# WardellZc/DeepLearningRecommendationSystem

Measured on AMD Instinct MI355X. Metric: CTR samples/sec fwd+bwd at batch 65536, higher is better.
Workload: dtype f32; 1 GPU; neuralcf mf_dim=64 layers=[128,64,32,16,8] users=943 items=1682 batch=65536/gpu (BASELINE configs[1]); global_batch=65536, parallelism=single

## Files before the change

### deeplearningrecommendationsystem_amd/csrc/ncf_proj.hip

```cpp
#include "ctr_common.h"

#include <stdlib.h>

namespace {

constexpr int kThreads = 256;
constexpr int kWaves = kThreads / 64;
constexpr int kL = 3;
constexpr int kK[kL] = {64, 32, 16};
constexpr int kN[kL] = {32, 16, 8};
constexpr int kH = 64;
constexpr int kN0 = 64;
constexpr int kP = 64;
constexpr int kNL = 8;
constexpr int kHeadW = kP + kNL;

#include "mfma16_tower.inc"

#ifdef CTR_STAMPS
__device__ unsigned long long g_stamps[2][64];
#define STAMP(k, i) do { const int at_ = (i); if (blockIdx.x == 7 && threadIdx.x == 0 && at_ < 64) g_stamps[k][at_] = __builtin_readcyclecounter(); } while (0)
#else
#define STAMP(k, i) do {} while (0)
#endif

struct Ids {
  const int64_t* uidx; int64_t ustride;
  const int64_t* iidx; int64_t istride;
  int64_t nu, ni;
};

constexpr int kChunks = 64;
constexpr int kPlanHead = 4;
static_assert(kPlanHead + 2 * (kChunks + 2) + 1 <= 2 * CTR_NCF_PROJ_COUNT_STRIDE,
              "CTR_NCF_PROJ_COUNT_STRIDE: the plan of the smallest tables (two rows) does not fit");
struct Plan {
  unsigned int* ticket;
  int32_t* base; int32_t* totals; int32_t* offsets;
  int64_t rows;
  int shift, chunks;
};
Plan plan_of(int32_t* buf, int64_t rows, int64_t m) {
  int shift = 8;
  while (((int64_t)kChunks << shift) < m) ++shift;
  Plan p;
  p.ticket = reinterpret_cast<unsigned int*>(buf);
  p.base = buf + kPlanHead;
  p.totals = p.base + kChunks * rows;
  p.offsets = p.totals + rows;
  p.rows = rows;
  p.shift = shift;
  p.chunks = (int)((m + ((int64_t)1 << shift) - 1) >> shift);
  return p;
}

struct RankJob {
  Ids ids;
  Plan plan; int32_t* ranks;
  int64_t m;
  int first;
};
constexpr int kRankPer = 4;
__device__ __forceinline__ void rank_role(const RankJob& R) {
  extern __shared__ __attribute__((aligned(16))) int s_hist[];
  const int chunk = (int)blockIdx.x - R.first;
  const int rows = (int)R.plan.rows;
  for (int i = threadIdx.x; i < rows; i += kThreads) s_hist[i] = 0;
  __syncthreads();
  const int64_t lo = (int64_t)chunk << R.plan.shift;
  const int64_t hi = lo + ((int64_t)1 << R.plan.shift) < R.m ? lo + ((int64_t)1 << R.plan.shift) : R.m;
  for (int64_t s0 = lo + threadIdx.x; s0 < hi; s0 += kRankPer * kThreads) {
    int64_t u[kRankPer], i[kRankPer];
#pragma unroll
    for (int e = 0; e < kRankPer; ++e) {
      const int64_t s = s0 + e * kThreads < hi ? s0 + e * kThreads : hi - 1;
      u[e] = R.ids.uidx[s * R.ids.ustride];
      i[e] = R.ids.iidx[s * R.ids.istride];
    }
#pragma unroll
    for (int e = 0; e < kRankPer; ++e) {
      const int64_t s = s0 + e * kThreads;
      if (s < hi) {
        int ru = -1, ri = -1;
        if ((uint64_t)u[e] < (uint64_t)R.ids.nu) ru = atomicAdd(s_hist + u[e], 1);
        if ((uint64_t)i[e] < (uint64_t)R.ids.ni) ri = atomicAdd(s_hist + R.ids.nu + i[e], 1);
        *reinterpret_cast<int2*>(R.ranks + 2 * s) = make_int2(ru, ri);
      }
    }
  }
  __syncthreads();
  int32_t* out = R.plan.base + (int64_t)chunk * rows;
  for (int i = threadIdx.x; i < rows; i += kThreads) out[i] = s_hist[i];
}

struct PlanJob {
  Plan plan;
  int first;
};
__device__ __forceinline__ void plan_role(const PlanJob& J, int* lds) {
  __shared__ int s_scan[kWaves];
  __shared__ bool s_last;
  const Plan& P = J.plan;
  const int64_t rows = P.rows;
  const int lane = threadIdx.x & 63, wave = threadIdx.x >> 6;
  {
    const int64_t row = ((int64_t)blockIdx.x - J.first) * kThreads + threadIdx.x;
    const int64_t rr = row < rows ? row : rows - 1;
    int v[kChunks];
#pragma unroll
    for (int c = 0; c < kChunks; ++c) v[c] = P.base[(int64_t)(c < P.chunks ? c : P.chunks - 1) * rows + rr];
    int run = 0;
#pragma unroll
    for (int c = 0; c < kChunks; ++c)
      if (c < P.chunks && row < rows) {
        P.base[(int64_t)c * rows + row] = run;
        run += v[c];
      }
    if (row < rows) __hip_atomic_store(P.totals + row, run, __ATOMIC_RELAXED, __HIP_MEMORY_SCOPE_AGENT);
  }
  __syncthreads();
  if (threadIdx.x == 0) {
    const unsigned int drawn = __hip_atomic_fetch_add(P.ticket, 1u, __ATOMIC_ACQ_REL, __HIP_MEMORY_SCOPE_AGENT);
    s_last = drawn == gridDim.x - (unsigned int)J.first - 1u;
  }
  __syncthreads();
  if (!s_last) return;
  constexpr int kCnt = 12;
  for (int64_t base = 0; base < rows; base += kCnt * kThreads) {
    int v[kCnt];
#pragma unroll
    for (int e = 0; e < kCnt; ++e) {
      const int64_t i = base + e * kThreads + threadIdx.x;
      v[e] = __hip_atomic_load(P.totals + (i < rows ? i : rows - 1), __ATOMIC_RELAXED, __HIP_MEMORY_SCOPE_AGENT);
    }
#pragma unroll
    for (int e = 0; e < kCnt; ++e) {
      const int64_t i = base + e * kThreads + threadIdx.x;
      if (i < rows) lds[i] = v[e];
    }
  }
  __syncthreads();
  const int per = (int)((rows + kThreads - 1) / kThreads);
  const int64_t i0 = (int64_t)threadIdx.x * per;
  int sum = 0;
  for (int e = 0; e < per; ++e)
    if (i0 + e < rows) sum += lds[i0 + e];
  int inc = sum;
#pragma unroll
  for (int d = 1; d < 64; d <<= 1) {
    const int v = __shfl_up(inc, d, 64);
    if (lane >= d) inc += v;
  }
  if (lane == 63) s_scan[wave] = inc;
  __syncthreads();
  int before = 0;
  for (int w = 0; w < wave; ++w) before += s_scan[w];
  int run = before + inc - sum;
  for (int e = 0; e < per; ++e)
    if (i0 + e < rows) {
      const int c = lds[i0 + e];
      lds[i0 + e] = run;
      run += c;
    }
  if (threadIdx.x == kThreads - 1) lds[rows] = before + inc;
  __syncthreads();
  for (int64_t i = threadIdx.x; i <= rows; i += kThreads) P.offsets[i] = lds[i];
  if (threadIdx.x == 0) __hip_atomic_store(P.ticket, 0u, __ATOMIC_RELAXED, __HIP_MEMORY_SCOPE_AGENT);
}

struct Prep {
  const float* mlp_u; const float* mlp_i;
  const float* w0; int64_t ldw0; const float* b0;
  float* ptab;
  int64_t nu, ni;
  const float* fold_u; const float* fold_w; int64_t fold_ldw; const float* fold_b; const float* fold_b2;
  float* wfold;
  RankJob rank;
};

__global__ void __launch_bounds__(kThreads)
ncfp_prep_kernel(const Prep A) {
  if ((int)blockIdx.x >= A.rank.first) {
    rank_role(A.rank);
    return;
  }
  const int lane = threadIdx.x & 63, q = lane >> 4, n = lane & 15;
  const int64_t wave = ((int64_t)blockIdx.x * kThreads + threadIdx.x) >> 6;
  const int64_t ublocks = (A.nu + 15) / 16, iblocks = (A.ni + 15) / 16;
  if ((int)blockIdx.x == A.rank.first - 1) {
    __shared__ float s_f[kThreads];
    const int t = threadIdx.x;
    const float* u = A.fold_u + kP;
    if (t < kP) A.wfold[t] = A.fold_u[t];
    {
      const int c = t & 7, i = t >> 3;
      s_f[t] = fmaf(A.fold_w[(int64_t)i * A.fold_ldw + c], u[i], A.fold_w[(int64_t)(i + 32) * A.fold_ldw + c] * u[i + 32]);
    }
    __syncthreads();
    if (t < kNL) {
      float acc = 0.0f;
      for (int i = 0; i < 32; ++i) acc += s_f[8 * i + t];
      A.wfold[kP + t] = acc;
    }
    __syncthreads();
    if (t < 64) s_f[t] = A.fold_b ? A.fold_b[t] * u[t] : 0.0f;
    __syncthreads();
    if (t == 0) {
      float acc = A.fold_b2 ? A.fold_b2[0] : 0.0f;
      for (int i = 0; i < 64; ++i) acc += s_f[i];
      A.wfold[kHeadW] = acc;
    }
  }
  if (wave >= ublocks + iblocks) return;
  const bool user = wave < ublocks;
  const int64_t row = (user ? wave : wave - ublocks) * 16 + n, rows = user ? A.nu : A.ni;
  const float* tab = user ? A.mlp_u : A.mlp_i;
  const int coff = user ? 0 : kH;
  const bool live = row < rows;
  f32x4 x[4], acc[4];
#pragma unroll
  for (int j = 0; j < 4; ++j) x[j] = ldg4(tab + (live ? row : 0) * kH + 16 * j + 4 * q);
#pragma unroll
  for (int b = 0; b < 4; ++b) {
    if (!user && A.b0) acc[b] = ldg4(A.b0 + 16 * b + 4 * q);
    else acc[b] = f32x4{0.f, 0.f, 0.f, 0.f};
  }
#pragma unroll
  for (int j = 0; j < 4; ++j) {
    f32x4 w[4];
#pragma unroll
    for (int b = 0; b < 4; ++b) w[b] = ldg4(A.w0 + (int64_t)(16 * b + n) * A.ldw0 + coff + 16 * j + 4 * q);
#pragma unroll
    for (int c = 0; c < 4; ++c)
#pragma unroll
      for (int b = 0; b < 4; ++b) acc[b] = __builtin_amdgcn_mfma_f32_16x16x4f32(w[b][c], x[j][c], acc[b], 0, 0, 0);
  }
  if (live) {
    float* dst = A.ptab + ((user ? 0 : A.nu) + row) * kN0 + 4 * q;
#pragma unroll
    for (int b = 0; b < 4; ++b) stg4(dst + 16 * b, acc[b]);
  }
}

struct Fwd {
  Ids ids;
  const float* ptab;
  const float* gmf_u; const float* gmf_i;
  const float* wfold;
  float* out; int64_t ldout; int act;
  int32_t* err_flag;
  PlanJob plan;
};

constexpr int kFwdStage = 4 * 16 * 64;
constexpr int kFwdStores = 5;

__global__ void __launch_bounds__(kThreads) __attribute__((amdgpu_waves_per_eu(2, 2)))
ncfp_fwd_kernel(const Tower T, int64_t m, const Fwd F) {
  extern __shared__ __attribute__((aligned(16))) float lds[];
  if ((int)blockIdx.x >= F.plan.first) {
    plan_role(F.plan, reinterpret_cast<int*>(lds));
    return;
  }
  float* s_w = lds;
  float* s_b = s_w + kWFloats;
  float* s_hw = s_b + kBFloats;
  const int lane = threadIdx.x & 63, q = lane >> 4, n = lane & 15;
  const int wave = __builtin_amdgcn_readfirstlane(threadIdx.x >> 6);
  float* stage = s_hw + 80 + wave * kFwdStage;
  const uint32_t stage_addr = ctr_lds_addr(stage);
  const int64_t groups = (m + 15) / 16;
  const int64_t wave0 = ((int64_t)blockIdx.x * kThreads + threadIdx.x) >> 6, nwaves = ((int64_t)F.plan.first * kThreads) >> 6;
  const uint32_t nu = (uint32_t)F.ids.nu, ni = (uint32_t)F.ids.ni;
  const float* tabs[4] = {F.ptab, F.ptab + F.ids.nu * kN0, F.gmf_u, F.gmf_i};
  int64_t idu = 0, idi = 0;
  auto issue_ids = [&](int64_t g) {
    int64_t row = g * 16 + n;
    row = row < m ? row : m - 1;
    idu = F.ids.uidx[row * F.ids.ustride];
    idi = F.ids.iidx[row * F.ids.istride];
  };
  auto issue_rows = [&](int64_t g) {
    const bool live = g * 16 + n < m;
    const bool ubad = (uint64_t)idu >= nu, ibad = (uint64_t)idi >= ni;
    const uint32_t u = ubad ? 0u : (uint32_t)idu, i = ibad ? 0u : (uint32_t)idi;
    if (live && (ubad || ibad) && F.err_flag) *F.err_flag = 1;
#pragma unroll
    for (int k = 0; k < 4; ++k) {
      const int r = 4 * k + q;
      const int src = (lane & 48) | r;
      const uint32_t ur = (uint32_t)__shfl((int)u, src, 64), ir = (uint32_t)__shfl((int)i, src, 64);
      const uint32_t col = 4u * (uint32_t)(n ^ r);
#pragma unroll
      for (int t = 0; t < 4; ++t) {
        const float* g_ = tabs[t] + ((t & 1) ? ir : ur) * 64u + col;
        ctr_dma16(g_, stage_addr + (uint32_t)((t * 16 + 4 * k) * 256));
      }
    }
  };
  auto staged = [&](int t, int j) {
    return *reinterpret_cast<const f32x4*>(stage + (t * 16 + n) * 64 + 4 * ((4 * j + q) ^ n));
  };
  int stamp = 0;
  (void)stamp;
  STAMP(0, stamp++);
  issue_ids(wave0);
  {
    f32x4 wv[kFStagePer];
    int wdst[kFStagePer];
    float bv;
    stage_forward_load(T, wv, wdst, bv);
    float hw = 0.0f;
    if (threadIdx.x <= kHeadW) hw = F.wfold[threadIdx.x];
    issue_rows(wave0);
    issue_ids(wave0 + nwaves);
    stage_forward_store(s_w, s_b, wv, wdst, bv);
    if (threadIdx.x <= kHeadW) s_hw[threadIdx.x] = hw;
  }
  __syncthreads();
  STAMP(0, stamp++);
  const float hc = s_hw[kHeadW];
  if (wave0 >= groups) return;
  asm volatile("s_waitcnt vmcnt(0)" ::: "memory");
  asm volatile("" : "+v"(idu), "+v"(idi));
  for (int64_t g = wave0; g < groups; g += nwaves) {
    const int64_t row = g * 16 + n;
    const int64_t srow = row < m ? row : m;
    f32x4 a0[4], xe[4];
#pragma unroll
    for (int j = 0; j < 4; ++j) {
      const f32x4 z = staged(0, j) + staged(1, j);
#pragma unroll
      for (int r = 0; r < 4; ++r) a0[j][r] = fmaxf(z[r], 0.0f);
    }
#pragma unroll
    for (int i = 0; i < 4; ++i)
      xe[i] = *reinterpret_cast<const f32x4*>(stage + (2 * 16 + n) * 64 + 4 * ((4 * q + i) ^ n)) *
              *reinterpret_cast<const f32x4*>(stage + (3 * 16 + n) * 64 + 4 * ((4 * q + i) ^ n));
    asm volatile("s_waitcnt lgkmcnt(0)" ::: "memory");
    STAMP(0, stamp++);
    issue_rows(g + nwaves);
    issue_ids(g + 2 * nwaves);
    STAMP(0, stamp++);
    f32x4 y1[2], y2[1], y3[1];
    layer_fwd<0, 4>(s_w, s_b, lane, q, a0, y1);
    layer_fwd<1, 2>(s_w, s_b, lane, q, y1, y2);
    layer_fwd<2, 1>(s_w, s_b, lane, q, y2, y3);
    STAMP(0, stamp++);
#pragma unroll
    for (int b = 0; b < 2; ++b) stg4(T.y[0] + srow * T.ldy[0] + 16 * b + 4 * q, y1[b]);
    stg4(T.y[1] + srow * T.ldy[1] + 4 * q, y2[0]);
    stg4(T.y[2] + (q < 2 ? srow : m) * T.ldy[2] + 4 * (q & 1), y3[0]);
    float dot = 0.0f;
#pragma unroll
    for (int i = 0; i < 4; ++i) {
      const f32x4 wv = *reinterpret_cast<const f32x4*>(s_hw + 16 * q + 4 * i);
      dot = fmaf(xe[i][0], wv[0], dot); dot = fmaf(xe[i][1], wv[1], dot);
      dot = fmaf(xe[i][2], wv[2], dot); dot = fmaf(xe[i][3], wv[3], dot);
    }
    {
      const f32x4 wv = *reinterpret_cast<const f32x4*>(s_hw + kP + 4 * (q & 1));
      float d2 = y3[0][0] * wv[0];
      d2 = fmaf(y3[0][1], wv[1], d2); d2 = fmaf(y3[0][2], wv[2], d2); d2 = fmaf(y3[0][3], wv[3], d2);
      dot += q < 2 ? d2 : 0.0f;
    }
    dot += __shfl_xor(dot, 16, 64);
    dot += __shfl_xor(dot, 32, 64);
    F.out[srow * F.ldout] = ctr_act(dot + hc, F.act);
    STAMP(0, stamp++);
    asm volatile("s_waitcnt vmcnt(%0)" ::"n"(kFwdStores) : "memory");
    asm volatile("" : "+v"(idu), "+v"(idi));
  }
}

constexpr int slab_w(int l) {
  int o = 0;
  for (int i = 0; i < l; ++i) o += kN[i] * kK[i] + kN[i];
  return o;
}
constexpr int kSlabHead = slab_w(kL);
constexpr int kVecs = 8 + 2 + 1;
constexpr int kSmall = 32 + 16 + 8 + 8 + 1;
constexpr int kCopy = kVecs * 256 + 68;
constexpr int kSlab = kCopy;
constexpr int kStripP = 3 * kTile;
constexpr int kSgPU = 0, kSgPI = 1024, kSgY1 = 2048, kSgY2 = 2560, kSgY3 = 2816, kBwdStage = 3072;
constexpr int kBwdLdsMax = 150 * 1024 / 4;
constexpr int64_t bwd_lds_floats(int64_t rows) {
  const int64_t main_f = kWFloats + kWaves * (kStripP + kBwdStage) + (rows + 1 + 3) / 4 * 4, copy_f = (int64_t)kWaves * kCopy;
  return main_f > copy_f ? main_f : copy_f;
}
static_assert(bwd_lds_floats(CTR_NCF_PROJ_MAX_ROWS) <= kBwdLdsMax, "CTR_NCF_PROJ_MAX_ROWS: the backward's offsets do not fit in LDS");
constexpr int kBwdDma = 12;
constexpr int kBwdStores = 6;

struct Bwd {
  Ids ids;
  const float* ptab;
  const float* wfold;
  const float* prob; int64_t ldp;
  const float* gprob; int64_t ldgp;
  int act;
  const int32_t* base;
  const int32_t* offsets;
  int shift;
  const int32_t* ranks;
  float* gz;
  float* aux;
  float* slabs;
  float* zero_a; int64_t zero_a_floats;
  float* zero_b; int64_t zero_b_floats;
};

__device__ __forceinline__ int sw1(int r) { return (r >> 1) & 7; }
__device__ __forceinline__ int sw2(int r) { return (r >> 2) & 3; }
__device__ __forceinline__ int sw3(int r) { return (r >> 3) & 1; }

__global__ void __launch_bounds__(kThreads)
ncfp_bwd_kernel(const Tower T, int64_t m, const Bwd B) {
  extern __shared__ __attribute__((aligned(16))) float lds[];
  __shared__ __attribute__((aligned(16))) float s_hw[kHeadW + 4];
  float* s_wt = lds;
  const int lane = threadIdx.x & 63, q = lane >> 4, lo = lane & 15;
  const int wave = __builtin_amdgcn_readfirstlane(threadIdx.x >> 6);
  float* tA = lds + kWFloats + wave * kStripP;
  float* tB = tA + 2 * kTile;
  float* stage = lds + kWFloats + kWaves * kStripP + wave * kBwdStage;
  const uint32_t stage_addr = ctr_lds_addr(stage);
  const int64_t nrows = B.ids.nu + B.ids.ni;
  int* s_off = reinterpret_cast<int*>(lds + kWFloats + kWaves * (kStripP + kBwdStage));
  const int64_t groups = (m + 15) / 16;
  const int64_t wave0 = ((int64_t)blockIdx.x * kThreads + threadIdx.x) >> 6, nwaves = ((int64_t)gridDim.x * kThreads) >> 6;
  const f32x4 zero4 = {0.f, 0.f, 0.f, 0.f};
  const float* pu = B.ptab;
  const float* pi = B.ptab + B.ids.nu * kN0;
  const uint32_t nu = (uint32_t)B.ids.nu, ni = (uint32_t)B.ids.ni;
  int stamp = 0;
  (void)stamp;
  STAMP(1, stamp++);

  {
    const int64_t t0 = ((int64_t)blockIdx.x * kThreads + threadIdx.x) * 4, step = (int64_t)gridDim.x * kThreads * 4;
    for (int64_t i = t0; i < B.zero_a_floats; i += step) stg4(B.zero_a + i, zero4);
    if (B.zero_b)
      for (int64_t i = t0; i < B.zero_b_floats; i += step) stg4(B.zero_b + i, zero4);
  }
  int64_t idu = 0, idi = 0;
  auto issue_ids = [&](int64_t g) {
    int64_t row = g * 16 + lo;
    row = row < m ? row : m - 1;
    idu = B.ids.uidx[row * B.ids.ustride];
    idi = B.ids.iidx[row * B.ids.istride];
  };
  struct Scal {
    float gp, pb;
    int ru, ri;
    int bu, bi;
    uint32_t u, i;
    bool ubad, ibad;
  };
  auto issue_rows = [&](int64_t g, Scal& r) {
    int64_t rc = g * 16 + lo;
    rc = rc < m ? rc : m - 1;
    r.ubad = (uint64_t)idu >= nu;
    r.ibad = (uint64_t)idi >= ni;
    r.u = r.ubad ? 0u : (uint32_t)idu;
    r.i = r.ibad ? 0u : (uint32_t)idi;
#pragma unroll
    for (int k = 0; k < 4; ++k) {
      const int row = 4 * k + q;
      const int src = (lane & 48) | row;
      const uint32_t ur = (uint32_t)__shfl((int)r.u, src, 64), ir = (uint32_t)__shfl((int)r.i, src, 64);
      const uint32_t col = 4u * (uint32_t)(lo ^ row);
      ctr_dma16(pu + ur * 64u + col, stage_addr + (uint32_t)((kSgPU + 4 * k * 64) * 4));
      ctr_dma16(pi + ir * 64u + col, stage_addr + (uint32_t)((kSgPI + 4 * k * 64) * 4));
    }
    {
      const int64_t g16 = g * 16;
#pragma unroll
      for (int k = 0; k < 2; ++k) {
        const int row = 8 * k + (lane >> 3);
        int64_t gr = g16 + row;
        gr = gr < m ? gr : m - 1;
        ctr_dma16(T.y[0] + gr * T.ldy[0] + 4 * ((lane & 7) ^ sw1(row)), stage_addr + (uint32_t)((kSgY1 + 8 * k * 32) * 4));
      }
      {
        const int row = lane >> 2;
        int64_t gr = g16 + row;
        gr = gr < m ? gr : m - 1;
        ctr_dma16(T.y[1] + gr * T.ldy[1] + 4 * ((lane & 3) ^ sw2(row)), stage_addr + (uint32_t)(kSgY2 * 4));
      }
      {
        const int row = (lane >> 1) & 15;
        int64_t gr = g16 + row;
        gr = gr < m ? gr : m - 1;
        ctr_dma16(T.y[2] + gr * T.ldy[2] + 4 * ((lane & 1) ^ sw3(row)), stage_addr + (uint32_t)(kSgY3 * 4));
      }
    }
    r.gp = B.gprob[rc * B.ldgp];
    r.pb = B.prob[rc * B.ldp];
    r.ru = B.ranks[2 * rc];
    r.ri = B.ranks[2 * rc + 1];
    const int32_t* bc = B.base + (rc >> B.shift) * nrows;
    r.bu = bc[r.u];
    r.bi = bc[nu + r.i];
  };
  Scal sc;
  f32x4 dw0[2][4], dw1[2], dw2;
  f32x4 sb0[2], sb1, sb2, hy = zero4;
  float hc = 0.0f;
#pragma unroll
  for (int b = 0; b < 2; ++b) {
    sb0[b] = zero4;
    dw1[b] = zero4;
#pragma unroll
    for (int j = 0; j < 4; ++j) dw0[b][j] = zero4;
  }
  sb1 = sb2 = dw2 = zero4;
  issue_ids(wave0);
  {
    f32x4 wv[kStagePer];
    int wdst[kStagePer];
    stage_transposed_load(T, wv, wdst);
    const float hw = threadIdx.x <= kHeadW ? B.wfold[threadIdx.x] : 0.0f;
    constexpr int kCnt = 12;
    for (int64_t base = 0; base <= nrows; base += kCnt * kThreads) {
      int v[kCnt];
#pragma unroll
      for (int e = 0; e < kCnt; ++e) {
        const int64_t i = base + e * kThreads + threadIdx.x;
        v[e] = B.offsets[i <= nrows ? i : nrows];
      }
#pragma unroll
      for (int e = 0; e < kCnt; ++e) {
        const int64_t i = base + e * kThreads + threadIdx.x;
        if (i <= nrows) s_off[i] = v[e];
      }
    }
    issue_rows(wave0, sc);
// ... 193 lines not shown
    for (int u = 0; u < 7; ++u) tail[u] = src[(int64_t)(p + 8 * u < A.parts ? p + 8 * u : A.parts - 1) * kSlab];
#pragma unroll
    for (int u = 0; u < 7; ++u) acc[0] += (p + 8 * u < A.parts ? 1.0f : 0.0f) * tail[u];
  }
  float t = ((acc[0] + acc[1]) + (acc[2] + acc[3])) + ((acc[4] + acc[5]) + (acc[6] + acc[7]));
  t += __shfl_xor(t, 32, 64);
  if ((threadIdx.x & 63) < 32) s_part[wave][o] = t;
  __syncthreads();
  if (threadIdx.x < 32 && e < kSlabHead) {
    const float total = (s_part[0][o] + s_part[1][o]) + (s_part[2][o] + s_part[3][o]);
    int l = 0, r = e;
#pragma unroll
    for (int i = 0; i < kL; ++i)
      if (e >= slab_w(i)) { l = i; r = e - slab_w(i); }
    const int wn = l == 0 ? kN[0] * kK[0] : l == 1 ? kN[1] * kK[1] : kN[2] * kK[2];
    float* dst = r < wn ? A.gw[l] + r : A.gb[l] + (r - wn);
    dst[0] += total;
  }
}

__device__ __forceinline__ void head_fold_role(const Seg& A) {
  __shared__ float s_p[28][12];
  __shared__ float s_g[12];
  const int col = threadIdx.x % 9, pl = threadIdx.x / 9;
  float acc = 0.0f;
  if (pl < 28) {
    const float* src = A.slabs + kVecs * 256 + 56 + col;
    float v[10];
#pragma unroll
    for (int u = 0; u < 10; ++u) v[u] = 0.0f;
    for (int p0 = pl; p0 < A.parts; p0 += 28 * 10) {
      float x[10];
#pragma unroll
      for (int u = 0; u < 10; ++u) x[u] = src[(int64_t)(p0 + 28 * u < A.parts ? p0 + 28 * u : A.parts - 1) * kSlab];
#pragma unroll
      for (int u = 0; u < 10; ++u) v[u] += (p0 + 28 * u < A.parts ? 1.0f : 0.0f) * x[u];
    }
#pragma unroll
    for (int u = 0; u < 10; ++u) acc += v[u];
    s_p[pl][col] = acc;
  }
  __syncthreads();
  if (threadIdx.x < 9) {
    float t = 0.0f;
    for (int i = 0; i < 28; ++i) t += s_p[i][threadIdx.x];
    s_g[threadIdx.x] = t;
  }
  __syncthreads();
  const float* u = A.fold_u + kP;
  const float gc = s_g[kNL];
  for (int t = threadIdx.x; t < 64 * kNL; t += kThreads) {
    const int i = t / kNL, q = t % kNL;
    if (A.g_w) A.g_w[(int64_t)i * A.ld_g_w + q] += u[i] * s_g[q];
  }
  if (threadIdx.x < 64) {
    const int i = threadIdx.x;
    if (A.g_u) {
      float sacc = A.fold_b ? A.fold_b[i] * gc : 0.0f;
#pragma unroll
      for (int q = 0; q < kNL; ++q) sacc = fmaf(A.fold_w[(int64_t)i * A.fold_ldw + q], s_g[q], sacc);
      A.g_u[kP + i] += sacc;
    }
    if (A.g_b) A.g_b[i] += u[i] * gc;
  }
  if (threadIdx.x == 64 && A.g_b2) A.g_b2[0] += gc;
}

constexpr int kSegSlots = 16;
constexpr int kSegGroups = kThreads / 16;
constexpr int kSegWgSlots = kSegGroups * kSegSlots;
constexpr int kSegOpenL = 1, kSegOpenR = 2;

__global__ void __launch_bounds__(kThreads, 3)
ncfp_segsum_kernel(const Seg A) {
  if ((int)blockIdx.x >= A.seg_blocks) {
    if ((int)blockIdx.x < A.seg_blocks + A.red_blocks) slab_reduce_role(A, (int)blockIdx.x - A.seg_blocks);
    else head_fold_role(A);
    return;
  }
  __shared__ __attribute__((aligned(16))) float s_run[2 * kSegGroups][128];
  __shared__ int s_meta[2 * kSegGroups];
  const int lane = threadIdx.x & 63, lo = lane & 15, grp = threadIdx.x >> 4;
  const int64_t s0 = ((int64_t)blockIdx.x * kSegGroups + grp) * kSegSlots, sme = s0 + lo;
  const int64_t spare = 2 * A.m;
  const int64_t total = A.offsets[A.nu + A.ni];
  const f32x4 rec = ldg4(A.aux + (sme < spare ? sme : spare) * 4);
  const int64_t sb = s0 > 0 ? s0 - 1 : 0, sa = s0 + kSegSlots;
  const int row_before = __float_as_int(A.aux[(sb < spare ? sb : spare) * 4 + 2]);
  const int row_after = __float_as_int(A.aux[(sa < spare ? sa : spare) * 4 + 2]);
  const bool used = sme < total;
  const float gzv = used ? rec[0] : 0.0f;
  const int v = used && (uint32_t)__float_as_int(rec[2]) < (uint32_t)(A.nu + A.ni) ? __float_as_int(rec[2]) : -1;
  const bool urow = v < A.nu;
  const uint32_t pid = used ? min((uint32_t)__float_as_int(rec[1]), (uint32_t)((urow ? A.ni : A.nu) - 1)) : 0u;
  const int pk = (int)(2u * pid + (urow ? 1u : 0u));
  const uint32_t b = used ? min((uint32_t)__float_as_int(rec[3]), (uint32_t)A.m) : (uint32_t)A.m;
  const int v_before = (s0 > 0 && s0 - 1 < total) ? row_before : -1;
  const int v_after = sa < total ? row_after : -1;
  f32x4 g[kSegSlots], p[kSegSlots];
#pragma unroll
  for (int k = 0; k < kSegSlots; ++k) {
    const int src = (lane & 48) | k;
    const uint32_t bk = (uint32_t)__shfl((int)b, src, 64);
    const int pkk = __shfl(pk, src, 64);
    g[k] = ldg4(A.gz + (int64_t)bk * kN0 + 4 * lo);
    p[k] = ldg4(((pkk & 1) ? A.gmf_i : A.gmf_u) + (int64_t)(pkk >> 1) * kP + 4 * lo);
  }
  const f32x4 zero4 = {0.f, 0.f, 0.f, 0.f};
  f32x4 accs = zero4, acct = zero4;
  int cur = -1;
  bool inside = false;
  int meta0 = -1, meta1 = -1;
  auto store_run = [&](int r) {
    float* dst = A.st + (int64_t)r * 128;
    stg4(dst + 4 * lo, accs);
    stg4(dst + 64 + 4 * lo, acct);
  };
  auto park = [&](int e) {
    *reinterpret_cast<f32x4*>(&s_run[2 * grp + e][4 * lo]) = accs;
    *reinterpret_cast<f32x4*>(&s_run[2 * grp + e][64 + 4 * lo]) = acct;
  };
#pragma unroll
  for (int k = 0; k < kSegSlots; ++k) {
    const int src = (lane & 48) | k;
    const int vk = __shfl(v, src, 64);
    const float gk = __shfl(gzv, src, 64);
    if (vk != cur) {
      if (cur >= 0) {
        if (inside) store_run(cur);
        else {
          park(0);
          meta0 = (cur << 2) | kSegOpenL;
        }
      }
      inside = k > 0 || vk != v_before;
      cur = vk;
      accs = acct = zero4;
    }
    accs += g[k];
    acct += gk * p[k];
  }
  if (cur >= 0) {
    const bool open_r = cur == v_after;
    if (inside && !open_r) store_run(cur);
    else {
      park(1);
      meta1 = (cur << 2) | (inside ? 0 : kSegOpenL) | (open_r ? kSegOpenR : 0);
    }
  }
  if (lo == 0) {
    s_meta[2 * grp] = meta0;
    s_meta[2 * grp + 1] = meta1;
  }
  __syncthreads();
  if (threadIdx.x >= 128) return;
  const int c = threadIdx.x;
  float sum = 0.0f;
  int row = -1;
  bool shared = false;
  auto emit = [&](bool atomic) {
    float* dst = A.st + (int64_t)row * 128 + c;
    if (atomic) ctr_atomic_add_global(dst, sum);
    else dst[0] = sum;
    row = -1;
  };
  int meta[2 * kSegGroups];
  float val[2 * kSegGroups];
#pragma unroll
  for (int e = 0; e < 2 * kSegGroups; ++e) {
    meta[e] = s_meta[e];
    val[e] = s_run[e][c];
  }
  asm volatile("" ::: "memory");
#pragma unroll
  for (int e = 0; e < 2 * kSegGroups; ++e) {
    const int mt = __builtin_amdgcn_readfirstlane(meta[e]);
    const float x = val[e];
    if (mt >= 0) {
      const int r = mt >> 2;
      if (row >= 0 && r != row) emit(true);
      if (row < 0) {
        row = r;
        sum = 0.0f;
        shared = (mt & kSegOpenL) != 0;
      }
      sum += x;
      if (!(mt & kSegOpenR)) emit(shared);
    }
  }
  if (row >= 0) emit(true);
}

struct Fin {
  const float* st;
  const float* mlp_u; const float* mlp_i; const float* gmf_u; const float* gmf_i;
  const float* w0; int64_t ldw0;
  const float* wfold;
  int64_t nu, ni;
  float* g_mlp_u; float* g_mlp_i; float* g_gmf_u; float* g_gmf_i;
  float* g_w0; int64_t ldgw0; float* g_b0;
  float* g_head;
  int wgs;
};
constexpr int kFinParts = 4;

__global__ void __launch_bounds__(kThreads)
ncfp_finish_kernel(const Fin A) {
  __shared__ __attribute__((aligned(16))) float s_dw[2][8 * 256];
  __shared__ float s_sm[kWaves][2][64];
  const int lane = threadIdx.x & 63, q = lane >> 4, n = lane & 15, wave = threadIdx.x >> 6;
  const int part = (int)blockIdx.x / A.wgs, wg = (int)blockIdx.x - part * A.wgs, h = part & 1;
  const int64_t ublocks = (A.nu + 15) / 16, iblocks = (A.ni + 15) / 16;
  const int64_t uwgs = (ublocks + kWaves - 1) / kWaves;
  const bool user = wg < uwgs;
  const int64_t blk = (user ? (int64_t)wg : (int64_t)wg - uwgs) * kWaves + wave;
  const int64_t rows = user ? A.nu : A.ni, r0 = blk * 16;
  const bool any = blk < (user ? ublocks : iblocks);
  const float* st = A.st + (user ? 0 : A.nu) * 128;
  const float* tab = user ? A.mlp_u : A.mlp_i;
  const float* gmf = user ? A.gmf_u : A.gmf_i;
  float* gtab = user ? A.g_mlp_u : A.g_mlp_i;
  float* ggmf = user ? A.g_gmf_u : A.g_gmf_i;
  const int coff = user ? 0 : kH;
  const f32x4 zero4 = {0.f, 0.f, 0.f, 0.f};
  const int64_t row = r0 + n;
  const bool live = any && row < rows;
  const int64_t crow = live ? row : rows - 1;
  const float keep = live ? 1.0f : 0.0f;

  if (part >= 2) {
    if (!any || (!gtab && !ggmf)) return;
    f32x4 sd[4], td[2], og[2], ot[2], wf[2];
    const float* ogp = ggmf ? ggmf : gmf;
    const float* otp = gtab ? gtab : tab;
#pragma unroll
    for (int j = 0; j < 4; ++j) sd[j] = ldg4(st + crow * 128 + 16 * j + 4 * q);
#pragma unroll
    for (int e = 0; e < 2; ++e) {
      const int col = 16 * (2 * h + e) + 4 * q;
      td[e] = ldg4(st + crow * 128 + 64 + col);
      og[e] = ldg4(ogp + crow * kP + col);
      ot[e] = ldg4(otp + crow * kH + col);
      wf[e] = ldg4(A.wfold + col);
    }
    f32x4 wt[4][2];
#pragma unroll
    for (int c = 0; c < 4; ++c)
#pragma unroll
      for (int e = 0; e < 2; ++e)
#pragma unroll
        for (int j = 0; j < 4; ++j) wt[j][e][c] = A.w0[(int64_t)(16 * j + 4 * q + c) * A.ldw0 + coff + 16 * (2 * h + e) + n];
    if (ggmf && live) {
#pragma unroll
      for (int e = 0; e < 2; ++e) stg4(ggmf + row * kP + 16 * (2 * h + e) + 4 * q, og[e] + wf[e] * td[e]);
    }
    if (gtab) {
#pragma unroll
      for (int j = 0; j < 4; ++j) sd[j] *= keep;
      f32x4 acc[2] = {ot[0], ot[1]};
#pragma unroll
      for (int j = 0; j < 4; ++j)
#pragma unroll
        for (int c = 0; c < 4; ++c)
#pragma unroll
          for (int e = 0; e < 2; ++e) acc[e] = __builtin_amdgcn_mfma_f32_16x16x4f32(wt[j][e][c], sd[j][c], acc[e], 0, 0, 0);
      if (live) {
#pragma unroll
        for (int e = 0; e < 2; ++e) stg4(gtab + row * kH + 16 * (2 * h + e) + 4 * q, acc[e]);
      }
    }
    return;
  }

  const bool sums = h == 0 && user && (A.g_b0 || A.g_head);
  if (!A.g_w0 && !sums) return;
  f32x4 dw[2][4];
#pragma unroll
  for (int e = 0; e < 2; ++e)
#pragma unroll
    for (int j = 0; j < 4; ++j) dw[e][j] = zero4;
  f32x4 colsum[4], gw[4];
#pragma unroll
  for (int j = 0; j < 4; ++j) colsum[j] = gw[j] = zero4;
  if (any) {
    f32x4 sd[4], td[4], gd[4];
#pragma unroll
    for (int j = 0; j < 4; ++j) {
      sd[j] = ldg4(st + crow * 128 + 16 * j + 4 * q);
      td[j] = ldg4(st + crow * 128 + 64 + 16 * j + 4 * q);
      gd[j] = ldg4(gmf + crow * kP + 16 * j + 4 * q);
    }
    f32x4 stt[2], xt[4];
    float okc[4];
#pragma unroll
    for (int c = 0; c < 4; ++c) {
      const int64_t r = r0 + 4 * q + c;
      const int64_t rr = r < rows ? r : rows - 1;
      okc[c] = r < rows ? 1.0f : 0.0f;
#pragma unroll
      for (int e = 0; e < 2; ++e) stt[e][c] = st[rr * 128 + 16 * (2 * h + e) + n];
#pragma unroll
      for (int j = 0; j < 4; ++j) xt[j][c] = tab[rr * kH + 16 * j + n];
    }
#pragma unroll
    for (int j = 0; j < 4; ++j) {
      gw[j] = gd[j] * (td[j] * keep);
      colsum[j] = sd[j] * keep;
    }
#pragma unroll
    for (int e = 0; e < 2; ++e)
#pragma unroll
      for (int c = 0; c < 4; ++c) stt[e][c] *= okc[c];
    if (A.g_w0) {
#pragma unroll
      for (int c = 0; c < 4; ++c)
#pragma unroll
        for (int e = 0; e < 2; ++e)
#pragma unroll
          for (int j = 0; j < 4; ++j) dw[e][j] = __builtin_amdgcn_mfma_f32_16x16x4f32(stt[e][c], xt[j][c], dw[e][j], 0, 0, 0);
    }
  }
  if (wave < 2) {
#pragma unroll
    for (int e = 0; e < 2; ++e)
#pragma unroll
      for (int j = 0; j < 4; ++j) *reinterpret_cast<f32x4*>(&s_dw[wave][((e * 4 + j) * 64 + lane) * 4]) = dw[e][j];
  }
  __syncthreads();
  if (wave >= 2) {
#pragma unroll
    for (int e = 0; e < 2; ++e)
#pragma unroll
      for (int j = 0; j < 4; ++j) {
        f32x4* at = reinterpret_cast<f32x4*>(&s_dw[wave - 2][((e * 4 + j) * 64 + lane) * 4]);
        *at = *at + dw[e][j];
      }
  }
  if (sums) {
#pragma unroll
    for (int j = 0; j < 4; ++j)
#pragma unroll
      for (int r = 0; r < 4; ++r) {
        const float cs = row_sum16(colsum[j][r]), gs = row_sum16(gw[j][r]);
        if (n == 0) {
          s_sm[wave][0][16 * j + 4 * q + r] = cs;
          s_sm[wave][1][16 * j + 4 * q + r] = gs;
        }
      }
  }
  __syncthreads();
  if (A.g_w0) {
    for (int e = threadIdx.x; e < 32 * 64; e += kThreads) {
      const int ul = e >> 6, k = e & 63, unit = 32 * h + ul;
      const int b = ul >> 4, qq = (ul >> 2) & 3, r = ul & 3, j = k >> 4, ll = k & 15;
      const int at = ((b * 4 + j) * 64 + qq * 16 + ll) * 4 + r;
      const float v = s_dw[0][at] + s_dw[1][at];
      ctr_atomic_add_global(A.g_w0 + (int64_t)unit * A.ldgw0 + coff + k, v);
    }
  }
  if (threadIdx.x < 64 && sums) {
    const int t = threadIdx.x;
    if (A.g_b0) ctr_atomic_add_global(A.g_b0 + t, (s_sm[0][0][t] + s_sm[1][0][t]) + (s_sm[2][0][t] + s_sm[3][0][t]));
    if (A.g_head) ctr_atomic_add_global(A.g_head + t, (s_sm[0][1][t] + s_sm[1][1][t]) + (s_sm[2][1][t] + s_sm[3][1][t]));
  }
}

int fill_tower(Tower* T, const ctr_mlp_layer_t* layers, bool need_y) {
  for (int l = 0; l < kL; ++l) {
    const ctr_mlp_layer_t& s = layers[l + 1];
    if (s.n != kN[l] || s.k != kK[l] || s.act != CTR_ACT_RELU || !s.w || !ctr_aligned16(s.w)) return CTR_ELIMIT;
    if (need_y && (!s.y || !ctr_aligned16(s.y) || s.ldy % 4 != 0 || s.ldy < s.n)) return CTR_ELIMIT;
    T->w[l] = s.w; T->b[l] = s.b; T->y[l] = s.y; T->ldy[l] = s.ldy;
  }
  return CTR_OK;
}

bool pattern_ok(const ctr_ncf_proj_t* d) {
  const ctr_mlp_layer_t& l0 = d->layers[0];
  return d->user_idx && d->item_idx && d->mlp_user && d->mlp_item && d->gmf_user && d->gmf_item && l0.w && l0.n == kN0 &&
         l0.k == 2 * kH && l0.act == CTR_ACT_RELU && ctr_aligned16(l0.w) && d->mlp_dim == kH && d->mf_dim == kP &&
         d->proj_n == kP && d->proj_k == kNL && d->proj_w && d->head_w && d->num_users >= 1 && d->num_items >= 1 &&
         d->num_users + d->num_items <= CTR_NCF_PROJ_MAX_ROWS && ctr_aligned16(d->mlp_user) && ctr_aligned16(d->mlp_item) &&
         ctr_aligned16(d->gmf_user) && ctr_aligned16(d->gmf_item) && d->ptab && ctr_aligned16(d->ptab) && d->wfold &&
         ctr_aligned16(d->wfold) && d->batch * 2 < ((int64_t)1 << 31);
}

}

#ifdef CTR_STAMPS
extern "C" __attribute__((visibility("default"))) int ctr_ncfp_debug_stamps(unsigned long long* out) {
  return (int)hipMemcpyFromSymbol(out, HIP_SYMBOL(g_stamps), sizeof(unsigned long long) * 128);
}
#endif

constexpr int kFwdWgs = 256;
constexpr int kBwdWgs = 256;
constexpr int kSlabsMax = 768;
static_assert(kBwdWgs <= kSlabsMax, "the backward's slabs must fit the workspace");

static int64_t workspace_floats(int64_t batch, int64_t num_users, int64_t num_items) {
  const int64_t rows = num_users + num_items;
  const int64_t groups = ctr_ceil_div(batch > 0 ? batch : 1, 16);
  int64_t grid = ctr_ceil_div(groups, kWaves);
  if (grid > kSlabsMax) grid = kSlabsMax;
  return (batch + 1) * kN0 + (2 * batch + 1) * 4 + rows * 128 + grid * (int64_t)kSlab;
}

extern "C" int ctr_ncf_proj_workspace_floats(int64_t batch, int64_t num_users, int64_t num_items, int64_t* floats) {
  CTR_REQUIRE(floats && batch >= 0 && num_users >= 0 && num_items >= 0, CTR_EINVAL);
  *floats = workspace_floats(batch, num_users, num_items);
  return CTR_OK;
}

extern "C" int ctr_ncf_proj_fwd(const ctr_ncf_proj_t* d, void* stream) {
  CTR_REQUIRE(d && d->batch >= 0, CTR_EINVAL);
  const int phases = d->phases ? d->phases : 3;
  if (!pattern_ok(d)) return CTR_ELIMIT;
  CTR_REQUIRE(d->prob && d->ldprob >= 1 && d->head_act >= CTR_ACT_NONE && d->head_act <= CTR_ACT_SIGMOID, CTR_EINVAL);
  CTR_REQUIRE(d->ld_proj_w >= d->proj_k, CTR_EINVAL);
  CTR_REQUIRE(!d->training || (d->plan && d->ranks), CTR_EINVAL);
  Tower T;
  int rc = fill_tower(&T, d->layers, true);
  if (rc != CTR_OK) return rc;
  hipStream_t st = (hipStream_t)stream;
  const int64_t nu = d->num_users, ni = d->num_items;
  const int64_t pwaves = ctr_ceil_div(nu, 16) + ctr_ceil_div(ni, 16);
  const Ids ids{d->user_idx, d->user_stride, d->item_idx, d->item_stride, nu, ni};
  const bool ranks = d->training && d->batch > 0;
  const Plan plan = plan_of(d->plan, nu + ni, d->batch);
  const int proj_blocks = (int)ctr_ceil_div(pwaves, kWaves) + 1;
  const Prep P{d->mlp_user, d->mlp_item, d->layers[0].w, d->layers[0].k, d->layers[0].b, d->ptab, nu, ni,
               d->head_w, d->proj_w, d->ld_proj_w, d->proj_b, d->head_b, d->wfold,
               RankJob{ids, plan, d->ranks, d->batch, proj_blocks}};
  const size_t prep_lds = ranks ? sizeof(int32_t) * (size_t)(nu + ni) : 0;
  if (hipFuncSetAttribute(reinterpret_cast<const void*>(ncfp_prep_kernel), hipFuncAttributeMaxDynamicSharedMemorySize,
                          (int)(sizeof(int32_t) * CTR_NCF_PROJ_MAX_ROWS)) != hipSuccess)
    return CTR_ELAUNCH;
  if (phases & 1)
    hipLaunchKernelGGL(ncfp_prep_kernel, dim3((unsigned)(proj_blocks + (ranks ? plan.chunks : 0))), dim3(kThreads), prep_lds, st, P);
  rc = ctr_launch_status();
  if (rc != CTR_OK || d->batch == 0 || !(phases & 2)) return rc;
  const int64_t groups = ctr_ceil_div(d->batch, 16);
  int64_t grid = ctr_ceil_div(groups, kWaves);
  if (grid > kFwdWgs) grid = kFwdWgs;
  const int64_t plan_blocks = ranks ? ctr_ceil_div(nu + ni, kThreads) : 0;
  const Fwd F{ids, d->ptab, d->gmf_user, d->gmf_item, d->wfold, d->prob, d->ldprob, d->head_act, d->err_flag,
              PlanJob{plan, (int)grid}};
  constexpr size_t fwd_lds = sizeof(float) * (kWFloats + kBFloats + 80 + kWaves * kFwdStage);
  static_assert(fwd_lds >= sizeof(int32_t) * (CTR_NCF_PROJ_MAX_ROWS + 1), "plan_role scans the offsets in the forward's LDS");
  if (hipFuncSetAttribute(reinterpret_cast<const void*>(ncfp_fwd_kernel), hipFuncAttributeMaxDynamicSharedMemorySize,
                          (int)fwd_lds) != hipSuccess)
    return CTR_ELAUNCH;
  hipLaunchKernelGGL(ncfp_fwd_kernel, dim3((unsigned)(grid + plan_blocks)), dim3(kThreads), fwd_lds, st, T, d->batch, F);
  return ctr_launch_status();
}

extern "C" int ctr_ncf_proj_bwd(const ctr_ncf_proj_t* d, const ctr_ncf_proj_grad_t* g, void* stream) {
  CTR_REQUIRE(d && g && d->batch >= 0, CTR_EINVAL);
  if (!pattern_ok(d)) return CTR_ELIMIT;
  CTR_REQUIRE(d->plan && d->ranks && d->prob && g->gprob && g->ldgprob >= 1 && g->workspace, CTR_EINVAL);
  CTR_REQUIRE(!g->zero_buf || (ctr_aligned16(g->zero_buf) && g->zero_floats % 4 == 0 && g->zero_floats >= 0), CTR_EALIGN);
  Tower T;
  int rc = fill_tower(&T, d->layers, true);
  if (rc != CTR_OK) return rc;
  hipStream_t st = (hipStream_t)stream;
  const int64_t m = d->batch, nu = d->num_users, ni = d->num_items, rows = nu + ni;
  if (m == 0) return g->zero_buf ? ctr_zero_fill(g->zero_buf, g->zero_floats, st) : CTR_OK;
  for (int l = 1; l <= kL; ++l) CTR_REQUIRE(g->layers[l].gw && g->layers[l].gb, CTR_EINVAL);
  CTR_REQUIRE(g->workspace_floats >= workspace_floats(m, nu, ni) && ctr_aligned16(g->workspace), CTR_ELIMIT);
  float* ws = g->workspace;
  float* gzb = ws;            ws += (m + 1) * kN0;
  float* aux = ws;            ws += (2 * m + 1) * 4;
  float* stt = ws;            ws += rows * 128;
  float* slabs = ws;
  const int64_t groups = ctr_ceil_div(m, 16);
  int64_t grid = ctr_ceil_div(groups, kWaves);
  if (grid > kBwdWgs) grid = kBwdWgs;
  const Ids ids{d->user_idx, d->user_stride, d->item_idx, d->item_stride, nu, ni};
  const Plan plan = plan_of(d->plan, rows, m);
  const int32_t* offs = plan.offsets;
  const Bwd B{ids, d->ptab, d->wfold, d->prob, d->ldprob, g->gprob, g->ldgprob, d->head_act, plan.base, offs, plan.shift,
              d->ranks, gzb, aux, slabs, stt, rows * 128, g->zero_buf, g->zero_buf ? g->zero_floats : 0};
  const size_t lds_bytes = sizeof(float) * (size_t)bwd_lds_floats(rows);
  CTR_REQUIRE(bwd_lds_floats(rows) <= kBwdLdsMax, CTR_ELIMIT);
  if (hipFuncSetAttribute(reinterpret_cast<const void*>(ncfp_bwd_kernel), hipFuncAttributeMaxDynamicSharedMemorySize,
                          (int)lds_bytes) != hipSuccess)
    return CTR_ELAUNCH;
  const int phases = g->phases ? g->phases : 7;
  if (phases & 1) hipLaunchKernelGGL(ncfp_bwd_kernel, dim3((unsigned)grid), dim3(kThreads), lds_bytes, st, T, m, B);
  rc = ctr_launch_status();
  if (rc != CTR_OK) return rc;
  Seg S{gzb, aux, offs, d->gmf_user, d->gmf_item, nu, ni, m, stt, (int)ctr_ceil_div(2 * m, kSegWgSlots),
        (kSlabHead + 31) / 32,
        slabs, (int)grid, {nullptr, nullptr, nullptr}, {nullptr, nullptr, nullptr}, d->head_w, d->proj_w, d->ld_proj_w,
        d->proj_b, g->g_head_w, g->g_proj_w, g->ld_g_proj_w, g->g_proj_b, g->g_head_b};
  for (int l = 0; l < kL; ++l) {
    S.gw[l] = g->layers[l + 1].gw;
    S.gb[l] = g->layers[l + 1].gb;
  }
  if (phases & 2)
    hipLaunchKernelGGL(ncfp_segsum_kernel, dim3((unsigned)(S.seg_blocks + S.red_blocks + 1)), dim3(kThreads), 0, st, S);
  rc = ctr_launch_status();
  if (rc != CTR_OK) return rc;
  const int64_t fwgs = ctr_ceil_div(ctr_ceil_div(nu, 16), kWaves) + ctr_ceil_div(ctr_ceil_div(ni, 16), kWaves);
  const Fin N{stt, d->mlp_user, d->mlp_item, d->gmf_user, d->gmf_item, d->layers[0].w, d->layers[0].k, d->wfold, nu, ni,
              g->g_mlp_user, g->g_mlp_item, g->g_gmf_user, g->g_gmf_item, g->layers[0].gw, d->layers[0].k, g->layers[0].gb,
              g->g_head_w, (int)fwgs};
  if (phases & 4) hipLaunchKernelGGL(ncfp_finish_kernel, dim3((unsigned)(kFinParts * fwgs)), dim3(kThreads), 0, st, N);
  return ctr_launch_status();
}
```

### deeplearningrecommendationsystem_amd/csrc/train_step.hip

```cpp
#include "ctr_common.h"

namespace {

constexpr int kBlock = 256;

__global__ void __launch_bounds__(kBlock)
bce_fwd_kernel(const float* __restrict__ p, int64_t ldp, const float* __restrict__ y, int64_t ldy, int64_t n,
               float inv_n, float* __restrict__ partial, unsigned int* __restrict__ ticket, float* __restrict__ loss,
               float* __restrict__ gp1 ) {
  __shared__ float s_red[kBlock / 64];
  __shared__ bool s_last;
  float acc = 0.0f;
  for (int64_t i = (int64_t)blockIdx.x * blockDim.x + threadIdx.x; i < n; i += (int64_t)gridDim.x * blockDim.x) {
    const float pv = p[i * ldp], yv = y[i * ldy];
    const float lp = fmaxf(logf(pv), -100.0f), l1p = fmaxf(logf(1.0f - pv), -100.0f);
    acc -= yv * lp + (1.0f - yv) * l1p;
    if (gp1) gp1[i] = (pv - yv) / fmaxf((1.0f - pv) * pv, 1e-12f) * inv_n;
  }
  acc = ctr_wave_sum(acc);
  if ((threadIdx.x & 63) == 0) s_red[threadIdx.x >> 6] = acc;
  __syncthreads();
  if (threadIdx.x == 0) {
    float t = 0.0f;
    for (int w = 0; w < kBlock / 64; ++w) t += s_red[w];
    __hip_atomic_store(partial + blockIdx.x, t * inv_n, __ATOMIC_RELAXED, __HIP_MEMORY_SCOPE_AGENT);
    const unsigned int drawn = __hip_atomic_fetch_add(ticket, 1u, __ATOMIC_ACQ_REL, __HIP_MEMORY_SCOPE_AGENT);
    s_last = drawn == gridDim.x - 1;
  }
  __syncthreads();
  if (!s_last) return;
  float v = threadIdx.x < gridDim.x
                ? __hip_atomic_load(partial + threadIdx.x, __ATOMIC_RELAXED, __HIP_MEMORY_SCOPE_AGENT)
                : 0.0f;
  v = ctr_wave_sum(v);
  if ((threadIdx.x & 63) == 0) s_red[threadIdx.x >> 6] = v;
  __syncthreads();
  if (threadIdx.x == 0) {
    float t = 0.0f;
    for (int w = 0; w < kBlock / 64; ++w) t += s_red[w];
    loss[0] = t;
    __hip_atomic_store(ticket, 0u, __ATOMIC_RELAXED, __HIP_MEMORY_SCOPE_AGENT);
  }
}

__global__ void __launch_bounds__(kBlock)
bce_bwd_kernel(const float* __restrict__ p, int64_t ldp, const float* __restrict__ y, int64_t ldy, int64_t n,
               const float* __restrict__ gloss, float inv_n, float* __restrict__ gp, int64_t ldg) {
  const float scale = gloss[0] * inv_n;
  for (int64_t i = (int64_t)blockIdx.x * blockDim.x + threadIdx.x; i < n; i += (int64_t)gridDim.x * blockDim.x) {
    const float pv = p[i * ldp], yv = y[i * ldy];
    gp[i * ldg] = (pv - yv) / fmaxf((1.0f - pv) * pv, 1e-12f) * scale;
  }
}

struct AdamPack {
  ctr_adam_tensor_t t[CTR_ADAM_MAX_TENSORS];
  int n;
};

__global__ void __launch_bounds__(kBlock)
adam_kernel(const AdamPack P, float lr, float beta2, float omb1, float omb2, float eps, float weight_decay, float bc1,
            float bc2_sqrt) {
  const ctr_adam_tensor_t t = P.t[blockIdx.y];
  const float step_size = lr / bc1;
  const bool near_end = omb1 >= 0.5f;
  const float b1 = 1.0f - omb1;
  for (int64_t i = ((int64_t)blockIdx.x * blockDim.x + threadIdx.x) * 4; i < t.numel; i += (int64_t)gridDim.x * blockDim.x * 4) {
    if (i + 3 < t.numel) {
      float4 g = *reinterpret_cast<const float4*>(t.grad + i);
      float4 p = *reinterpret_cast<const float4*>(t.param + i);
      float4 m = *reinterpret_cast<const float4*>(t.exp_avg + i);
      float4 v = *reinterpret_cast<const float4*>(t.exp_avg_sq + i);
      float* gg = &g.x; float* pp = &p.x; float* mm = &m.x; float* vv = &v.x;
#pragma unroll
      for (int e = 0; e < 4; ++e) {
        const float gr = fmaf(weight_decay, pp[e], gg[e]);
        mm[e] = near_end ? fmaf(mm[e] - gr, b1, gr) : fmaf(omb1, gr - mm[e], mm[e]);
        vv[e] = vv[e] * beta2 + (omb2 * gr) * gr;
        const float denom = sqrtf(vv[e]) / bc2_sqrt + eps;
        pp[e] -= step_size * (mm[e] / denom);
      }
      *reinterpret_cast<float4*>(t.param + i) = p;
      *reinterpret_cast<float4*>(t.exp_avg + i) = m;
      *reinterpret_cast<float4*>(t.exp_avg_sq + i) = v;
    } else {
      for (int64_t j = i; j < t.numel; ++j) {
        const float gr = fmaf(weight_decay, t.param[j], t.grad[j]);
        const float m = near_end ? fmaf(t.exp_avg[j] - gr, b1, gr) : fmaf(omb1, gr - t.exp_avg[j], t.exp_avg[j]);
        const float v = t.exp_avg_sq[j] * beta2 + (omb2 * gr) * gr;
        t.exp_avg[j] = m;
        t.exp_avg_sq[j] = v;
        t.param[j] -= step_size * (m / (sqrtf(v) / bc2_sqrt + eps));
      }
    }
  }
}

}

extern "C" int ctr_bce_fwd(const float* prob, int64_t ldp, const float* target, int64_t ldt, int64_t n, float* loss,
                           float* workspace, int64_t workspace_floats, unsigned int* ticket, float* gprob_unit,
                           void* stream) {
  CTR_REQUIRE(n > 0 && prob && target && loss && workspace && ticket && ldp >= 1 && ldt >= 1, CTR_EINVAL);
  int64_t grid = ctr_ceil_div(n, kBlock * 4);
  if (grid > 256) grid = 256;
  CTR_REQUIRE(workspace_floats >= grid, CTR_ELIMIT);
  hipLaunchKernelGGL(bce_fwd_kernel, dim3((unsigned)grid), dim3(kBlock), 0, (hipStream_t)stream, prob, ldp, target, ldt,
                     n, 1.0f / (float)n, workspace, ticket, loss, gprob_unit);
  return ctr_launch_status();
}

extern "C" int ctr_bce_bwd(const float* prob, int64_t ldp, const float* target, int64_t ldt, int64_t n,
                           const float* gloss, float* gprob, int64_t ldg, void* stream) {
  CTR_REQUIRE(n > 0 && prob && target && gloss && gprob && ldp >= 1 && ldt >= 1 && ldg >= 1, CTR_EINVAL);
  hipLaunchKernelGGL(bce_bwd_kernel, dim3(ctr_stream_grid(n, kBlock)), dim3(kBlock), 0, (hipStream_t)stream, prob, ldp,
                     target, ldt, n, gloss, 1.0f / (float)n, gprob, ldg);
  return ctr_launch_status();
}

extern "C" int ctr_adam_step(const ctr_adam_tensor_t* tensors, int ntensors, double lr, double beta1, double beta2,
                             double eps, double weight_decay, int64_t step, void* stream) {
  CTR_REQUIRE(tensors && ntensors >= 0 && step >= 1, CTR_EINVAL);
  const double bc1 = 1.0 - pow(beta1, (double)step);
  const double bc2 = 1.0 - pow(beta2, (double)step);
  hipStream_t st = (hipStream_t)stream;
  for (int base = 0; base < ntensors; base += CTR_ADAM_MAX_TENSORS) {
    AdamPack P;
    P.n = ntensors - base < CTR_ADAM_MAX_TENSORS ? ntensors - base : CTR_ADAM_MAX_TENSORS;
    int64_t longest = 0;
    for (int i = 0; i < P.n; ++i) {
      const ctr_adam_tensor_t& t = tensors[base + i];
      CTR_REQUIRE(t.param && t.grad && t.exp_avg && t.exp_avg_sq && t.numel >= 0, CTR_EINVAL);
      CTR_REQUIRE(ctr_aligned16(t.param) && ctr_aligned16(t.grad) && ctr_aligned16(t.exp_avg) &&
                      ctr_aligned16(t.exp_avg_sq),
                  CTR_EALIGN);
      P.t[i] = t;
      longest = t.numel > longest ? t.numel : longest;
    }
    if (longest == 0) continue;
    int64_t gx = ctr_ceil_div(longest, kBlock * 4);
    if (gx > 2048) gx = 2048;
    hipLaunchKernelGGL(adam_kernel, dim3((unsigned)gx, (unsigned)P.n), dim3(kBlock), 0, st, P, (float)lr,
                       (float)beta2, (float)(1.0 - beta1), (float)(1.0 - beta2), (float)eps, (float)weight_decay,
                       (float)bc1, (float)sqrt(bc2));
    int rc = ctr_launch_status();
    if (rc != CTR_OK) return rc;
  }
  return CTR_OK;
}
```

Before: 913.9 million samples/s.

## Batch loads ahead of use and relax ticket atomics to acquire-only on last block

```diff
diff --git a/deeplearningrecommendationsystem_amd/csrc/ncf_proj.hip b/deeplearningrecommendationsystem_amd/csrc/ncf_proj.hip
--- a/deeplearningrecommendationsystem_amd/csrc/ncf_proj.hip
+++ b/deeplearningrecommendationsystem_amd/csrc/ncf_proj.hip
@@ -118,10 +118,16 @@
       }
     if (row < rows) __hip_atomic_store(P.totals + row, run, __ATOMIC_RELAXED, __HIP_MEMORY_SCOPE_AGENT);
   }
+  asm volatile("s_waitcnt vmcnt(0)" ::: "memory");
   __syncthreads();
   if (threadIdx.x == 0) {
-    const unsigned int drawn = __hip_atomic_fetch_add(P.ticket, 1u, __ATOMIC_ACQ_REL, __HIP_MEMORY_SCOPE_AGENT);
-    s_last = drawn == gridDim.x - (unsigned int)J.first - 1u;
+    const unsigned int drawn = __hip_atomic_fetch_add(P.ticket, 1u, __ATOMIC_RELAXED, __HIP_MEMORY_SCOPE_AGENT);
+    const bool last = drawn == gridDim.x - (unsigned int)J.first - 1u;
+    s_last = last;
+    if (last) {
+      __builtin_amdgcn_fence(__ATOMIC_ACQUIRE, "agent");
+      asm volatile("s_waitcnt vmcnt(0)" ::: "memory");
+    }
   }
   __syncthreads();
   if (!s_last) return;
@@ -217,24 +223,29 @@
   const float* tab = user ? A.mlp_u : A.mlp_i;
   const int coff = user ? 0 : kH;
   const bool live = row < rows;
-  f32x4 x[4], acc[4];
+  f32x4 x[4], w[4][4], acc[4];
+  const bool biased = !user && A.b0;
+  const float* bias = A.b0 ? A.b0 : A.w0;
 #pragma unroll
   for (int j = 0; j < 4; ++j) x[j] = ldg4(tab + (live ? row : 0) * kH + 16 * j + 4 * q);
 #pragma unroll
-  for (int b = 0; b < 4; ++b) {
-    if (!user && A.b0) acc[b] = ldg4(A.b0 + 16 * b + 4 * q);
-    else acc[b] = f32x4{0.f, 0.f, 0.f, 0.f};
-  }
-#pragma unroll
-  for (int j = 0; j < 4; ++j) {
-    f32x4 w[4];
-#pragma unroll
-    for (int b = 0; b < 4; ++b) w[b] = ldg4(A.w0 + (int64_t)(16 * b + n) * A.ldw0 + coff + 16 * j + 4 * q);
+  for (int j = 0; j < 4; ++j)
+#pragma unroll
+    for (int b = 0; b < 4; ++b) w[j][b] = ldg4(A.w0 + (int64_t)(16 * b + n) * A.ldw0 + coff + 16 * j + 4 * q);
+#pragma unroll
+  for (int b = 0; b < 4; ++b) acc[b] = ldg4(bias + 16 * b + 4 * q);
+  asm volatile("" : "+v"(x[0]), "+v"(x[1]), "+v"(x[2]), "+v"(x[3]), "+v"(acc[0]), "+v"(acc[1]), "+v"(acc[2]), "+v"(acc[3]),
+                    "+v"(w[0][0]), "+v"(w[0][1]), "+v"(w[0][2]), "+v"(w[0][3]), "+v"(w[1][0]), "+v"(w[1][1]), "+v"(w[1][2]),
+                    "+v"(w[1][3]), "+v"(w[2][0]), "+v"(w[2][1]), "+v"(w[2][2]), "+v"(w[2][3]), "+v"(w[3][0]), "+v"(w[3][1]),
+                    "+v"(w[3][2]), "+v"(w[3][3]));
+#pragma unroll
+  for (int b = 0; b < 4; ++b) acc[b] = biased ? acc[b] : f32x4{0.f, 0.f, 0.f, 0.f};
+#pragma unroll
+  for (int j = 0; j < 4; ++j)
 #pragma unroll
     for (int c = 0; c < 4; ++c)
 #pragma unroll
-      for (int b = 0; b < 4; ++b) acc[b] = __builtin_amdgcn_mfma_f32_16x16x4f32(w[b][c], x[j][c], acc[b], 0, 0, 0);
-  }
+      for (int b = 0; b < 4; ++b) acc[b] = __builtin_amdgcn_mfma_f32_16x16x4f32(w[j][b][c], x[j][c], acc[b], 0, 0, 0);
   if (live) {
     float* dst = A.ptab + ((user ? 0 : A.nu) + row) * kN0 + 4 * q;
 #pragma unroll
@@ -1034,6 +1045,9 @@
 #pragma unroll
       for (int j = 0; j < 4; ++j) xt[j][c] = tab[rr * kH + 16 * j + n];
     }
+    asm volatile("" : "+v"(sd[0]), "+v"(sd[1]), "+v"(sd[2]), "+v"(sd[3]), "+v"(td[0]), "+v"(td[1]), "+v"(td[2]), "+v"(td[3]),
+                      "+v"(gd[0]), "+v"(gd[1]), "+v"(gd[2]), "+v"(gd[3]), "+v"(stt[0]), "+v"(stt[1]), "+v"(xt[0]), "+v"(xt[1]),
+                      "+v"(xt[2]), "+v"(xt[3]));
 #pragma unroll
     for (int j = 0; j < 4; ++j) {
       gw[j] = gd[j] * (td[j] * keep);
diff --git a/deeplearningrecommendationsystem_amd/csrc/train_step.hip b/deeplearningrecommendationsystem_amd/csrc/train_step.hip
--- a/deeplearningrecommendationsystem_amd/csrc/train_step.hip
+++ b/deeplearningrecommendationsystem_amd/csrc/train_step.hip
@@ -3,6 +3,35 @@
 namespace {
 
 constexpr int kBlock = 256;
+constexpr int kBceFly = 4;
+
+struct BceBlock {
+  float p[kBceFly], y[kBceFly];
+};
+__device__ __forceinline__ void bce_request(BceBlock& v, const float* __restrict__ p, int64_t ldp, const float* __restrict__ y,
+                                            int64_t ldy, int64_t first, int64_t stride, int64_t n) {
+#pragma unroll
+  for (int e = 0; e < kBceFly; ++e) {
+    const int64_t i = first + e * stride, ic = i < n ? i : n - 1;
+    v.p[e] = p[ic * ldp];
+    v.y[e] = y[ic * ldy];
+  }
+}
+__device__ __forceinline__ void bce_consume(BceBlock& v, int64_t first, int64_t stride, int64_t n, float inv_n,
+                                            float* __restrict__ gp1, float& acc) {
+  asm volatile("" : "+v"(v.p[0]), "+v"(v.p[1]), "+v"(v.p[2]), "+v"(v.p[3]), "+v"(v.y[0]), "+v"(v.y[1]), "+v"(v.y[2]), "+v"(v.y[3]));
+  static_assert(kBceFly == 4, "the pin above names every element");
+#pragma unroll
+  for (int e = 0; e < kBceFly; ++e) {
+    const int64_t i = first + e * stride;
+    const bool live = i < n;
+    const float pv = v.p[e], yv = v.y[e];
+    const float lp = fmaxf(logf(pv), -100.0f), l1p = fmaxf(logf(1.0f - pv), -100.0f);
+    const float sub = acc - (yv * lp + (1.0f - yv) * l1p);
+    acc = live ? sub : acc;
+    if (gp1 && live) gp1[i] = (pv - yv) / fmaxf((1.0f - pv) * pv, 1e-12f) * inv_n;
+  }
+}
 
 __global__ void __launch_bounds__(kBlock)
 bce_fwd_kernel(const float* __restrict__ p, int64_t ldp, const float* __restrict__ y, int64_t ldy, int64_t n,
@@ -10,12 +39,12 @@
                float* __restrict__ gp1 ) {
   __shared__ float s_red[kBlock / 64];
   __shared__ bool s_last;
+  const int64_t stride = (int64_t)gridDim.x * blockDim.x, i0 = (int64_t)blockIdx.x * blockDim.x + threadIdx.x;
   float acc = 0.0f;
-  for (int64_t i = (int64_t)blockIdx.x * blockDim.x + threadIdx.x; i < n; i += (int64_t)gridDim.x * blockDim.x) {
-    const float pv = p[i * ldp], yv = y[i * ldy];
-    const float lp = fmaxf(logf(pv), -100.0f), l1p = fmaxf(logf(1.0f - pv), -100.0f);
-    acc -= yv * lp + (1.0f - yv) * l1p;
-    if (gp1) gp1[i] = (pv - yv) / fmaxf((1.0f - pv) * pv, 1e-12f) * inv_n;
+  for (int64_t base = 0; base < n; base += kBceFly * stride) {
+    BceBlock v;
+    bce_request(v, p, ldp, y, ldy, i0 + base, stride, n);
+    bce_consume(v, i0 + base, stride, n, inv_n, gp1, acc);
   }
   acc = ctr_wave_sum(acc);
   if ((threadIdx.x & 63) == 0) s_red[threadIdx.x >> 6] = acc;
@@ -24,8 +53,14 @@
     float t = 0.0f;
     for (int w = 0; w < kBlock / 64; ++w) t += s_red[w];
     __hip_atomic_store(partial + blockIdx.x, t * inv_n, __ATOMIC_RELAXED, __HIP_MEMORY_SCOPE_AGENT);
-    const unsigned int drawn = __hip_atomic_fetch_add(ticket, 1u, __ATOMIC_ACQ_REL, __HIP_MEMORY_SCOPE_AGENT);
-    s_last = drawn == gridDim.x - 1;
+    asm volatile("s_waitcnt vmcnt(0)" ::: "memory");
+    const unsigned int drawn = __hip_atomic_fetch_add(ticket, 1u, __ATOMIC_RELAXED, __HIP_MEMORY_SCOPE_AGENT);
+    const bool last = drawn == gridDim.x - 1;
+    s_last = last;
+    if (last) {
+      __builtin_amdgcn_fence(__ATOMIC_ACQUIRE, "agent");
+      asm volatile("s_waitcnt vmcnt(0)" ::: "memory");
+    }
   }
   __syncthreads();
   if (!s_last) return;
```

Measured after the change: 938.2 million samples/s, median of 6. 1.03x the previous value.
